# bab2min/Kiwi

Measured on AMD Instinct MI355X. Metric: sentences/sec on batched analyze(), device kernels with inputs resident in HBM (dictionary scan + lattice + Viterbi/Knlm, top-1); host-to-host rate: see e2e, higher is better.
Workload: dtype int32+f32; 1 GPU; c2-64k: 65536 synthetic sentences ({'exact_jamo': 40}), synthetic 'full' model (kiwi_amd/synth.py), Knlm, top-1; sentences_per_gpu=65536, chunks_per_gpu=65536, jamo_per_gpu=2621440, parallelism=shard1, device_bytes=9402884427, rerun_chunks=0

## Files before the change

### kiwi_amd/csrc/engine.hip

```cpp
#include <hip/hip_runtime.h>
#include <unistd.h>
#include <cstdio>
#include <cstring>
#include <ctime>
#include <algorithm>
#include <atomic>
#include <cstdlib>
#include <chrono>
#include <condition_variable>
#include <functional>
#include <map>
#include <mutex>
#include <numeric>
#include <stdexcept>
#include <thread>
#include "engine.hpp"
#include "pretok.hpp"
#include "hostpool.hpp"
#include "post_fast.hpp"
#include "viterbi_kernel.hpp"
#include "exact_math.hpp"
#include "cong_global.hpp"
#include "chr_freq.hpp"
#include "typo_lattice_kernel.hpp"
// ... 31 lines not shown
				size_t best = blocks.size();
				for (size_t i = 0; i < blocks.size(); ++i)
					if (blocks[i].device == device && blocks[i].cap >= n && blocks[i].cap <= 2 * n + (1u << 20) && (best == blocks.size() || blocks[i].cap < blocks[best].cap)) best = i;
				if (best == blocks.size()) return nullptr;
				void* p = blocks[best].p; capOut = blocks[best].cap; bytes -= capOut;
				blocks.erase(blocks.begin() + best);
				return p;
			}
			void give(void* p, size_t cap, int device)
			{
				{
					std::lock_guard<std::mutex> g{ mu };
					if (blocks.size() < kMaxBlocks && bytes + cap <= kMaxBytes) { blocks.push_back(Block{ p, cap, device }); bytes += cap; return; }
				}
				release(Block{ p, cap, device });
			}
			void trim()
			{
				std::lock_guard<std::mutex> g{ mu };
				for (auto& b : blocks) release(b);
				blocks.clear(); bytes = 0;
			}
		};
		DevBlockCache& devCache() { static DevBlockCache c; return c; }
		int currentDevice() { int d = 0; (void)hipGetDevice(&d); return d; }

		struct DevBuf
		{
			void* p = nullptr; size_t cap = 0; int device = 0;
			DevBuf() = default;
			DevBuf(const DevBuf&) = delete;
			DevBuf& operator=(const DevBuf&) = delete;
			~DevBuf() { release(); }
			void release() { if (p) devCache().give(p, cap, device); p = nullptr; cap = 0; }
			void ensure(size_t n)
			{
				if (n <= cap) return;
				release();
				device = currentDevice();
				const size_t want = n + n / 8 + 256;
				p = devCache().take(want, cap, device);
				if (!p)
				{
					hipError_t e = hipMalloc(&p, want);
					if (e == hipErrorOutOfMemory) { (void)hipGetLastError(); devCache().trim(); e = hipMalloc(&p, want); }
					if (e != hipSuccess) { p = nullptr; (void)hipGetLastError(); throw std::runtime_error{ std::string{ "HIP error in hipMalloc(" } + std::to_string(want) + " bytes): " + hipGetErrorString(e) }; }
					cap = want;
// ... 2363 lines not shown
```

### kiwi_amd/csrc/viterbi_pos.inc

```
#if !defined(KAMD_SBG) && !defined(KAMD_CONGG)
	template<int G> struct PosCaps
	{
#ifdef KAMD_TEST_SMALL_CAPS
		static constexpr uint32_t PST_CAP = 8;
#else
		static constexpr uint32_t PST_CAP = G == 16 ? 64 : 32;
#endif
		static constexpr uint32_t PHR = G == 16 ? 32 : 16;
	};
	constexpr uint32_t PBIG_CAP = 64;
	struct PosGroupCtx { uint64_t st, recs, uniq, nodeTypo; uint32_t stCap, stTop, posStart, ringTop, firstRec, retry, ofNodes, pad; };
	static_assert(sizeof(PosGroupCtx) == 64, "PosGroupCtx");
	template<int G> struct PosLayT
	{
		static constexpr uint32_t PST_CAP = PosCaps<G>::PST_CAP, PHR = PosCaps<G>::PHR;
		static constexpr uint32_t RBEG = 0, REND = 4 * RING, RCUM = 8 * RING;
		static constexpr uint32_t NCNT = 12 * RING;
		static constexpr uint32_t ACUR = NCNT + 4 * G, ALAST = ACUR + 32, ATMP = ALAST + 32;
#ifdef KAMD_TEST_DEAD_WINDOW
		static constexpr uint32_t DWIN_BITS = KAMD_TEST_DEAD_WINDOW;
#else
		static constexpr uint32_t DWIN_BITS = 256;
#endif
		static constexpr uint32_t DWIN = ATMP + 32, DWIN_WORDS = DWIN_BITS / 32;
		static constexpr uint32_t GCTX = DWIN + (G == 16 ? 32 : 0);
		static constexpr uint32_t RINFO = GCTX + 64;
		static constexpr uint32_t PBEST = RINFO;
		static constexpr uint32_t OVFL = RINFO + 4 * G;
		static constexpr uint32_t RECS = OVFL + 16;
		static constexpr uint32_t STSC = RECS + G * 48;
		static constexpr uint32_t STB = STSC + 4 * PST_CAP;
		static constexpr uint32_t HOTR = (STB + 2 * PST_CAP + 15) & ~15u;
		static constexpr uint32_t TYPR = HOTR + 16 * PHR;
#ifdef KAMD_CONG
// ... 80 lines not shown
	}
	__device__ __forceinline__ uint32_t nthSetBit(uint32_t v, uint32_t k)
	{
		uint32_t pos = 0, c;
		c = (uint32_t)__popc(v & 0xFFFFu); if (k >= c) { k -= c; pos += 16; v >>= 16; }
		c = (uint32_t)__popc(v & 0xFFu); if (k >= c) { k -= c; pos += 8; v >>= 8; }
		c = (uint32_t)__popc(v & 0xFu); if (k >= c) { k -= c; pos += 4; v >>= 4; }
		c = (uint32_t)__popc(v & 0x3u); if (k >= c) { k -= c; pos += 2; v >>= 2; }
		if (k >= (v & 1u)) pos += 1;
		return pos;
	}
	__device__ __forceinline__ void ldsMaxF(LDS_AS float* p, float v)
	{
#if defined(__HIP_DEVICE_COMPILE__)
		__hip_atomic_fetch_max(p, v, __ATOMIC_RELAXED, __HIP_MEMORY_SCOPE_WAVEFRONT);
#else
		uint32_t o = __atomic_load_n((uint32_t*)p, __ATOMIC_RELAXED);
		while (v > __uint_as_float(o) && !__atomic_compare_exchange_n((uint32_t*)p, &o, __float_as_uint(v), false, __ATOMIC_RELAXED, __ATOMIC_RELAXED)) {}
#endif
	}

	struct PosKernArgs { ModelView M; BatchView B; WorkView W; SearchParams P; const uint32_t* chunkOrder; uint32_t nWork; TYPO_ONLY(const float* nodeTypoAll;) CONG_ONLY(CongDev CG;) };
#ifdef KAMD_HIPEMU
	__device__ __noinline__ bool continueChunk(const PosKernArgs* A, uint32_t chunk, uint32_t gl, uint32_t grp, uint32_t slot, uint32_t resumeAt, const uint8_t* scratchCheck, const uint32_t* orderCheck, uint32_t nWorkCheck)
	{
#else
	__device__ __noinline__ bool continueChunk(uint32_t chunk, uint32_t gl, uint32_t grp, uint32_t slot, uint32_t resumeAt, const uint8_t* scratchCheck, const uint32_t* orderCheck, uint32_t nWorkCheck)
	{
		const PosKernArgs* A = (const PosKernArgs*)((const uint8_t*)__builtin_amdgcn_implicitarg_ptr() - ((sizeof(PosKernArgs) + 7) & ~(size_t)7));
#endif
		if (A->W.posScratch != scratchCheck || A->chunkOrder != orderCheck || A->nWork != nWorkCheck) return false;
		const ModelView& M = A->M; const SearchParams& P = A->P; const BatchView& B = A->B; const WorkView& W = A->W;
		CONG_ONLY(const CongDev& CG = A->CG;)
		GroupCtx<16> X(M, P);
		X.gl = gl; X.gshift = grp * 16; X.lds = grp * Lay<16>::SIZE;
		X.scratch = reinterpret_cast<GroupScratch*>(W.posScratch) + slot;
		X.tl = nullptr;
		TYPO_ONLY(X.typoAll = A->nodeTypoAll; X.nodeTypo = nullptr;)
		CONG_ONLY(X.CG = &CG; X.outFirst = false;)
		searchChunk<16>(X, B, W, chunk, resumeAt);
		return true;
	}

	template<int G, int WPS>
	__global__ void __launch_bounds__(64, WPS) k_pos_path(ModelView M, BatchView B, WorkView W, SearchParams P, const uint32_t* chunkOrder, uint32_t nWork TYPO_ONLY(, const float* nodeTypoAll) CONG_ONLY(, CongDev CGv))
	{
		static_assert(G == 16 || G == 8, "a lane group is one DPP row or half of one");
		using PosLay = PosLayT<G>;
		constexpr uint32_t NG = 64 / G, GM = (1u << G) - 1u, PST_CAP = PosLay::PST_CAP, PHR = PosLay::PHR;
		constexpr bool kLiveOnly = G == 16;
#ifdef KAMD_TYPO
		constexpr uint32_t kP = 2;
#else
		constexpr uint32_t kP = 16 / G;
#endif
		const uint32_t lane = threadIdx.x, gl = lane & (uint32_t)(G - 1), gshift = lane & (uint32_t)(64 - G), grp = lane / (uint32_t)G, lds = grp * PosLay::SIZE;
		const uint32_t il = lane & 15u, irow = lane >> 4;
		LDS_AS uint32_t* rBeg = ldsPtr<uint32_t>(lds + PosLay::RBEG);
		LDS_AS uint32_t* rEnd = ldsPtr<uint32_t>(lds + PosLay::REND);
		LDS_AS uint32_t* rCum = ldsPtr<uint32_t>(lds + PosLay::RCUM);
		LDS_AS uint32_t* nCnt = ldsPtr<uint32_t>(lds + PosLay::NCNT);
		LDS_AS uint32_t* aCur = ldsPtr<uint32_t>(lds + PosLay::ACUR);
		LDS_AS uint32_t* aLast = ldsPtr<uint32_t>(lds + PosLay::ALAST);
		LDS_AS uint32_t* aTmp = ldsPtr<uint32_t>(lds + PosLay::ATMP);
// ... 16 lines not shown
#define GBALLOT(p) ((uint32_t)((__ballot(p) >> gshift) & GM))
#define GSHFL(v, l) __shfl((v), (int)(l), G)
#ifdef KAMD_HIPEMU
#define WBALLOT(p) hipemu_ballot64(p)
#define WSHFL(v, l) hipemu_shfl64((v), (int)(l))
#define WREADLANE(v, l) hipemu_shfl64((v), (int)(l))
#define IROR(N, v) ((uint32_t)hipemu_row_ror64((int)(v), (N)))
#define IRORF(N, v) __uint_as_float((uint32_t)hipemu_row_ror64((int)__float_as_uint(v), (N)))
#else
#define WBALLOT(p) ((unsigned long long)__ballot(p))
#define WSHFL(v, l) __shfl((v), (int)(l), 64)
#define WREADLANE(v, l) ((uint32_t)__builtin_amdgcn_readlane((int)(v), (int)(l)))
#define IROR(N, v) rowRor<N>(v)
#define IRORF(N, v) rowRorF<N>(v)
#endif
#ifdef KAMD_POS_DEBUG
#define PBEACON(code, a, b2, c2) { if (W.beacon && mine && gl == 0) { uint32_t* bq_ = W.beacon + 64ull * chunk; __builtin_nontemporal_store((uint32_t)(code), bq_); __builtin_nontemporal_store((uint32_t)(a), bq_ + 1); __builtin_nontemporal_store((uint32_t)(b2), bq_ + 2); __builtin_nontemporal_store((uint32_t)(c2), bq_ + 3); } }
		unsigned long long tlLast = clock64(); uint32_t tlAcc[14] = { 0, 0, 0, 0, 0, 0, 0, 0, 0, 0, 0, 0, 0, 0 };
#define PTL(k) { const unsigned long long t_ = clock64(); tlAcc[k] += (uint32_t)(t_ - tlLast); tlLast = t_; }
#else
#define PBEACON(code, a, b2, c2)
#define PTL(k)
#endif
		const unsigned long long lowerMask64 = (1ull << lane) - 1ull;

		const uint32_t ci = blockIdx.x * NG + grp;
		const bool mine = ci < nWork;
		const uint32_t chunk = mine ? chunkOrder[ci] : chunkOrder[0];
		DevChunkResult* res = &W.results[chunk];
		bool active = mine && res->status == CS_OK;
		if (mine && !active && gl == 0) res->nPaths = 0;
		const bool searching = active;
		PBEACON(1, ci, 0, 0)
		const uint32_t nBase = W.nodeBase[chunk];
		const uint32_t Gn = W.nNodes[chunk];
		DevState* st = W.states + W.stateBase[chunk];
		const uint32_t stCap = (uint32_t)(W.stateBase[chunk + 1] - W.stateBase[chunk]);
		uint32_t* nodeStOff = W.nodeStateOff + nBase; uint32_t* nodeStCnt = W.nodeStateCnt + nBase; uint16_t* nodeLive = W.tmpIdx + 2ull * nBase;
		const uint8_t* uniq = B.spStates + B.spOff[chunk];
		uint8_t* reach = W.reach + nBase;
		const PosDesc* desc = W.posDesc + nBase;
		const PosRec* recs = W.posRecs + W.packBase[chunk];
		const uint32_t* posPrev = W.posPrev + nBase;
#ifdef KAMD_TYPO
		const float* nodeTypo = nodeTypoAll + nBase;
#else
		const float* nodeTypo = nullptr;
#endif
		const uint32_t nPos = active ? desc[0].firstRec : 0u, eosStart = active ? desc[0].pad2 : 0u;
		const uint32_t* posStarts = W.posMask + nBase;
		TYPO_ONLY(const uint32_t* posStarts2 = posStarts + W.nodeBase[B.nChunks];)
		const bool canPropagate = nPos <= 255 && active && desc[0].nNodes == 0;
		bool scanned = false;
		if (gl < 8) { aCur[gl] = gl == 0 ? 1u : 0u; aLast[gl] = 0; if constexpr (kLiveOnly) ldsPtr<uint32_t>(lds + PosLay::DWIN)[gl] = 0; }
		for (uint32_t k = gl; k < 16; k += G) gctx[k] = 0;
		rinfo[gl] = 0; if (gl == 0) *ovfL = 0;

		uint32_t stTop = 1, cumLive = 1;
		uint32_t ringTop = 1;
		uint32_t stopAt = 0;
		if (active)
		{
			if (gl == 0)
			{
				const MorphRec m0 = M.morphs[0];
				storeState(st, 0, M.h.bosNode, 0.f, 0.f, 0, m0.feat, COMMON_ROOT, 0, 0, m0.prevFlags, 0, 0xFFFFFFFFu, 0, 0.f, 0, 0);
				nodeStOff[0] = 0; nodeStCnt[0] = 1; nodeLive[0] = 1;
				rBeg[0] = 0; rEnd[0] = 1; rCum[0] = 1;
				ldsStore4(hotR, make_uint4((uint32_t)M.h.bosNode, 0u, (uint32_t)m0.feat | ((uint32_t)COMMON_ROOT << 16), (uint32_t)m0.prevFlags << 8));
				typR[0] = 0.f;
#ifdef KAMD_CONG
				ctxR[0] = 0;
#else
				const uint32_t c1 = M.lmChain[2 * (uint32_t)M.h.bosNode], c2 = M.lmChain[2 * (uint32_t)M.h.bosNode + 1];
				chR[0] = c1; chR[1] = c2;
				*reinterpret_cast<uint2*>(&st[0].pad0) = make_uint2(c1, c2);
#endif
			}
			for (uint32_t k = gl; k < Gn; k += G) reach[k] = k == 0 ? 1 : 0;
			if (!nPos) { stopAt = 1u | (8u << 24); active = false; }
		}

		uint4 dqA = make_uint4(0, 0, 0, 0), dqB = make_uint4(0, 0, 0, 0);
		uint32_t ppA = 0, rqA = 0;
		uint4 recA0 = make_uint4(0, 0, 0, 0), recA1 = recA0, recA2 = recA0, recB0 = recA0, recB1 = recA0, recB2 = recA0;
		if (active)
		{
			dqA = *reinterpret_cast<const uint4*>(desc + 1);
			if (nPos >= 2) dqB = *reinterpret_cast<const uint4*>(desc + 2);
			if (gl < ((dqA.x >> 16) & 0xFFu)) ppA = posPrev[(dqA.x & 0xFFFFu) + gl];
			if (gl < (dqA.z & 0xFFFFu)) rqA = recs[dqA.y + gl].rq;
			if constexpr (WPS <= 2) if (gl < (dqA.z & 0xFFFFu)) { const uint4* rp0 = reinterpret_cast<const uint4*>(recs + dqA.y + gl); recA0 = rp0[0]; recA1 = rp0[1]; recA2 = rp0[2]; }
		}

		uint32_t pi = 1, attempt = 0, retry0 = 0, retry1 = 0;
		uint4 dqC = make_uint4(0, 0, 0, 0); uint32_t ppB = 0, rqB = 0;
		uint32_t guardSteps = 0;
		__syncthreads();

		while (WBALLOT(active))
		{
			if (++guardSteps > 4u * 0x10000u) break;
			if (lane == 0) PSTAT(0, 1)
			if (gl == 0 && active) PSTAT(1, 1)
			const uint4 dq = dqA;
			const uint32_t i0 = dq.x & 0xFFFFu, m = (dq.x >> 16) & 0xFFu, firstRec = dq.y, nRec = dq.z & 0xFFFFu;
			uint32_t Qp[kP]; uint32_t rqp[kP], pBegRp[kP];
#pragma unroll
			for (uint32_t ps_ = 0; ps_ < kP; ++ps_) { Qp[ps_] = 0; rqp[ps_] = 0; pBegRp[ps_] = 0; }
			uint32_t posStart = stTop;
			CONG_ONLY(uint32_t ofNodes = 0;)
			uint4 rec0 = recA0, rec1 = recA1, rec2 = recA2;
			if (active)
			{
				PBEACON(2, pi, i0, (m << 16) | nRec)
				PTL(0)
				if ((dq.x >> 24) || m > (uint32_t)G || nRec > kP * (uint32_t)G) { stopAt = i0 | (1u << 24); active = false; }
			}
			if (active)
			{
				if (!attempt)
				{
					dqC = make_uint4(0, 0, 0, 0); ppB = 0; rqB = 0;
					if (pi + 2 <= nPos) dqC = *reinterpret_cast<const uint4*>(desc + pi + 2);
					if (pi + 1 <= nPos)
					{
						if (gl < ((dqB.x >> 16) & 0xFFu)) ppB = posPrev[(dqB.x & 0xFFFFu) + gl];
						if (gl < (dqB.z & 0xFFFFu)) rqB = recs[dqB.y + gl].rq;
						if constexpr (WPS <= 2) if (gl < (dqB.z & 0xFFFFu)) { const uint4* rp0 = reinterpret_cast<const uint4*>(recs + dqB.y + gl); recB0 = rp0[0]; recB1 = rp0[1]; recB2 = rp0[2]; }
					}
				}
				if constexpr (WPS > 2) if (gl < nRec) { const uint4* rp0 = reinterpret_cast<const uint4*>(recs + firstRec + gl); rec0 = rp0[0]; rec1 = rp0[1]; rec2 = rp0[2]; }
				rqp[0] = rqA;
				if constexpr (kP > 1) if (nRec > (uint32_t)G && gl + G < nRec) rqp[kP - 1] = recs[firstRec + G + gl].rq;
				uint32_t pBeg = 0, nP = 0, nLv = 0; bool bad = false; uint32_t why = 0;
				if (gl < m)
				{
					const uint32_t fp = ppA & 0xFFFFu, lp = fp + ((ppA >> 16) & 0xFFu);
					if (i0 + gl - fp + 1 >= RING) { bad = true; why = 2; }
					else
					{
						pBeg = rBeg[fp & (RING - 1)];
						nP = rEnd[lp & (RING - 1)] - pBeg;
						const uint32_t nLive = rCum[lp & (RING - 1)] - (fp ? rCum[(fp - 1) & (RING - 1)] : 0u);
						if (nLive > P.smallMax) { bad = true; why = 3; }
						nLv = nLive;
					}
				}
				nCnt[gl] = 0;
				if (gl == 0) { PHIST(0, nRec) PHIST(1, m) }
#pragma unroll
				for (uint32_t ps_ = 0; ps_ < kP; ++ps_)
				{
					const uint32_t rq = rqp[ps_];
					const uint32_t nlR = (rq >> 8) & 0xFFu, Rr = rq & 0xFFu;
					const uint32_t nPk = GSHFL(kLiveOnly ? nLv : nP, nlR), pBegR = GSHFL(pBeg, nlR);
					const uint32_t Q = ps_ * G + gl < nRec ? nPk * Rr : 0u;
#if defined(KAMD_POSSTATS) && defined(KAMD_HIPEMU)
					{ const uint32_t nAll = GSHFL(nP, nlR); if (kLiveOnly && ps_ * G + gl < nRec && !bad) PSTAT(5, (nAll - nPk) * Rr) }
#endif
					if (Q > PBIG_CAP || pBegR >= (1u << 27)) { bad = true; why = 4; }
					Qp[ps_] = Q; pBegRp[ps_] = pBegR;
					if (ps_ * G + gl < nRec) PHIST(3, Q)
				}
				if (gl < m && !bad) PHIST(5, i0 + gl - (ppA & 0xFFFFu))
				if (GBALLOT(bad)) { stopAt = i0 | (grpMaxU<G>(why) << 24); active = false; }
#ifdef KAMD_CONG
				if (active)
				{
					uint32_t wantL = 0;
#pragma unroll
					for (uint32_t ps_ = 0; ps_ < kP; ++ps_)
					{
						const uint32_t rq = rqp[ps_], nlR = (rq >> 8) & 0xFFu;
						const uint32_t nPk = GSHFL(nP, nlR);
						if (ps_ * G + gl < nRec && (rq & PR_OUT_FIRST) && nPk >= 4) wantL |= 1u << nlR;
					}
					const uint32_t want = grpOr<G>(wantL);
					for (uint32_t wn = want; wn; wn &= wn - 1)
					{
						const uint32_t j = (uint32_t)__ffs((int)wn) - 1u;
						const uint32_t pb = GSHFL(pBeg, j), np = GSHFL(nP, j);
						if (G < 16 || np > 16)
						{
							static_assert(4 * PBIG_CAP <= G * 48, "context list in the record area");
							LDS_AS uint32_t* cxs = ldsPtr<uint32_t>(lds + PosLay::RECS);
							for (uint32_t b = 0; b < np; b += G)
							{
								const uint32_t k = b + gl;
								if (k < np) { const Hot h = loadHot(st, pb + k); cxs[k] = (!h.dead() && !h.socket()) ? st[pb + k].pad0 : 0xFFFFFFFFu; }
							}
							waveSyncLds();
							uint32_t mu = 0;
							for (uint32_t b = 0; b < np; b += G)
							{
								const uint32_t k = b + gl;
								bool isNew = false;
								if (k < np)
								{
									const uint32_t cx = cxs[k];
									isNew = cx != 0xFFFFFFFFu;
// ... 7 lines not shown
						}
						if constexpr (G == 16)
						{
						uint32_t cx = 0xFFFFFFFFu; bool ok = false;
						if (gl < np) { const Hot h = loadHot(st, pb + gl); ok = !h.dead() && !h.socket(); cx = st[pb + gl].pad0; }
						const uint32_t okw = ok ? 1u : 0u;
						bool isNew = ok;
#define KAMD_UNIQ_STEP(N) { const uint32_t oc = rowRor<N>(cx), oo = rowRor<N>(okw); isNew = isNew & !((oo != 0) & (oc == cx) & (((gl - N) & 15u) < gl)); }
						KAMD_UNIQ_STEP(1) KAMD_UNIQ_STEP(2) KAMD_UNIQ_STEP(3) KAMD_UNIQ_STEP(4) KAMD_UNIQ_STEP(5) KAMD_UNIQ_STEP(6) KAMD_UNIQ_STEP(7) KAMD_UNIQ_STEP(8)
						KAMD_UNIQ_STEP(9) KAMD_UNIQ_STEP(10) KAMD_UNIQ_STEP(11) KAMD_UNIQ_STEP(12) KAMD_UNIQ_STEP(13) KAMD_UNIQ_STEP(14) KAMD_UNIQ_STEP(15)
#undef KAMD_UNIQ_STEP
						const uint32_t mu = (uint32_t)__popc(GBALLOT(isNew));
						if (mu >= 4 && mu != 8) ofNodes |= 1u << j;
						}
					}
				}
#endif
				if (active)
				{
					rinfo[gl] = pBegRp[0] | ((rqp[0] & 0xFFu) << 27);
					if (gl < nRec) { ldsStore4(lds + PosLay::RECS + 48 * gl, rec0); ldsStore4(lds + PosLay::RECS + 48 * gl + 16, rec1); ldsStore4(lds + PosLay::RECS + 48 * gl + 32, rec2); }
					if (gl == 0)
					{
						LDS_AS uint64_t* g64 = (LDS_AS uint64_t*)gctx;
						g64[0] = (uint64_t)st; g64[1] = (uint64_t)(recs + firstRec); g64[2] = (uint64_t)uniq; g64[3] = (uint64_t)nodeTypo;
						gctx[8] = stCap; gctx[9] = stTop; gctx[10] = stTop; gctx[11] = ringTop; gctx[12] = 0; gctx[13] = retry0 | (retry1 << 16);
#ifdef KAMD_CONG
						gctx[14] = ofNodes;
#else
						gctx[14] = 0;
#endif
						gctx[15] = 0;
						*ovfL = 0;
					}
					posStart = stTop;
				}
				PTL(1)
			}
			__syncthreads();

			for (uint32_t pass = 0; pass < kP; ++pass)
			{
			if (pass)
			{
				if (!WBALLOT(active && nRec > (uint32_t)G)) break;
				if (active)
				{
					rinfo[gl] = pBegRp[kP - 1] | ((rqp[kP - 1] & 0xFFu) << 27);
					if (G + gl < nRec)
					{
						const uint4* rp0 = reinterpret_cast<const uint4*>(recs + firstRec + G + gl);
						ldsStore4(lds + PosLay::RECS + 48 * gl, rp0[0]); ldsStore4(lds + PosLay::RECS + 48 * gl + 16, rp0[1]); ldsStore4(lds + PosLay::RECS + 48 * gl + 32, rp0[2]);
					}
				}
				__syncthreads();
			}
			const uint32_t Qw = active ? ((kP > 1 && pass) ? Qp[kP - 1] : Qp[0]) : 0u;

			{
				uint32_t S16 = Qw;
				{ uint32_t t; t = IROR(1, S16); S16 += il >= 1 ? t : 0u; t = IROR(2, S16); S16 += il >= 2 ? t : 0u; t = IROR(4, S16); S16 += il >= 4 ? t : 0u; t = IROR(8, S16); S16 += il >= 8 ? t : 0u; }
				const uint32_t T0 = WREADLANE(S16, 15), T1 = WREADLANE(S16, 31), T2 = WREADLANE(S16, 47);
				const uint32_t Winc = S16 + (irow >= 1 ? T0 : 0u) + (irow >= 2 ? T1 : 0u) + (irow >= 3 ? T2 : 0u);
				const unsigned long long nzAll = WBALLOT(Qw != 0);
				uint32_t recDoneW = 0, baseW = 0, guardW = 0;
				while (recDoneW < 64)
				{
					const unsigned long long nz = nzAll & ~((1ull << recDoneW) - 1ull);
					if (!nz) break;
					if (++guardW > 80u) { *ovfL = 1; break; }
					const bool take = lane >= recDoneW && Winc - baseW <= 64u;
					const uint32_t n = (uint32_t)__popcll(WBALLOT(take));
					if (!n) { *ovfL = 1; break; }
					const uint32_t nItems = WREADLANE(Winc, recDoneW + n - 1) - baseW;
// ... 382 lines not shown
				}
				waveSyncLds();
				const bool scanRoots = GBALLOT(otherRoot) != 0;
				for (uint32_t b = 0; b < cnt; b += G)
				{
					const uint32_t i = b + gl;
					if (i >= cnt) continue;
					const uint32_t bits = stB[i]; const float lim = stSc[i] + P.cutOff;
					bool kill = lim < pbest[(bits >> 8) & 0xFu];
					if (scanRoots && (bits & 0x1Fu))
					{
						kill = false;
						for (uint32_t j = 0; j < cnt; ++j)
						{
							const uint32_t bj = stB[j];
							if (!(bj & SB_MORPH_SOCKET) && (bj & 0xF1Fu) == (bits & 0xF1Fu) && lim < stSc[j]) kill = true;
						}
					}
					if constexpr (kLiveOnly)
					{
						LDS_AS uint32_t* dwp = ldsPtr<uint32_t>(lds + PosLay::DWIN) + (((posStart + i) >> 5) & (PosLay::DWIN_WORDS - 1u));
						if (kill) ldsOr(dwp, 1u << ((posStart + i) & 31u)); else ldsAnd(dwp, ~(1u << ((posStart + i) & 31u)));
					}
					if (kill) { st[posStart + i].dead = 1; if (ringTop - (posStart + i) <= PHR) ldsPtr<uint32_t>(hotR + 16 * ((posStart + i) & (PHR - 1)) + 12)[0] |= 1u << 16; }
					ldsAdd(&nCnt[(bits >> 8) & 0xFu], 1u | ((bits & PSB_PASS1) ? 0u : 1u << 8) | (kill ? 0u : 1u << 16) | ((kill || (bits & SB_STATE_SOCKET)) ? 0u : 1u << 24));
				}
				waveSyncLds();
				PTL(8)
				const uint32_t myC = nCnt[gl];
				const uint32_t myCnt = myC & 0xFFu, myP0 = (myC >> 8) & 0xFFu, myLive = (myC >> 16) & 0xFFu, myFree = myC >> 24;
				const bool isNode = gl < m, formNode = isNode && !((dq.z >> (16 + gl)) & 1u);
				bool redo = false;
				if (attempt == 0)
				{
					const uint32_t lacking = GBALLOT(isNode && !myP0);
					if (lacking) { retry0 = lacking; attempt = 1; redo = true; }
				}
				if (!redo && attempt <= 1)
				{
					const uint32_t stateless = GBALLOT(isNode && !myCnt && ((dq.w >> gl) & 1u));
					if (stateless) { retry0 |= stateless; retry1 = stateless; attempt = 2; redo = true; }
				}
				if (redo && gl == 0) PSTAT(13, 1)
				if (redo) stTop = posStart;
				else
				{
				const uint32_t spJ = ppA >> 24;
// ... 3 lines not shown
				if (!nonFree) flagBits = GBALLOT(isNode && (formNode || tbit(aLast, spJ)));
				else
				{
					if (!canPropagate) { stopAt = i0 | (9u << 24); active = false; }
					else
					{
					const bool predFlag = isNode && tbit(aCur, spJ);
					flagBits = 0; bool disconnected = false;
					for (uint32_t j = 0; j < m; ++j)
					{
						const uint32_t spj = GSHFL(spJ, j);
						if (!((nonFree >> j) & 1u))
						{
							if (!((dq.z >> (16 + j)) & 1u) || tbit(aLast, spj)) flagBits |= 1u << j;
							continue;
						}
						const uint32_t later = GBALLOT(predFlag && gl > j);
						if (gl < 8) aTmp[gl] = aCur[gl];
						waveSyncLds();
						if (flagBits || later) sbit(aTmp, pi);
						for (uint32_t x = pi + 1; x <= nPos; x += G)
						{
							uint32_t st4 = 0; TYPO_ONLY(uint32_t st8 = 0;)
							if (x + gl <= nPos) { st4 = posStarts[x + gl]; TYPO_ONLY(st8 = posStarts2[x + gl];) }
							const uint32_t nx = nPos - x + 1 < (uint32_t)G ? nPos - x + 1 : (uint32_t)G;
							for (uint32_t t = 0; t < nx; ++t)
							{
								const uint32_t s4 = GSHFL(st4, t);
								uint32_t reached = tbit(aTmp, s4 & 0xFFu) | tbit(aTmp, (s4 >> 8) & 0xFFu) | tbit(aTmp, (s4 >> 16) & 0xFFu) | tbit(aTmp, s4 >> 24);
								TYPO_ONLY({ const uint32_t s8 = GSHFL(st8, t); reached |= tbit(aTmp, s8 & 0xFFu) | tbit(aTmp, (s8 >> 8) & 0xFFu) | tbit(aTmp, (s8 >> 16) & 0xFFu) | tbit(aTmp, s8 >> 24); })
								if (reached) sbit(aTmp, x + t);
							}
						}
						if (!tbit(aTmp, eosStart)) { disconnected = true; break; }
						waveSyncLds();
						if (gl < 8) aLast[gl] = aTmp[gl];
						waveSyncLds();
						scanned = true;
					}
					if (disconnected) { stopAt = i0 | (7u << 24); active = false; }
					}
				}

				if (active)
				{
				if (flagBits) sbit(aCur, pi);
				PTL(9)
				PBEACON(10, pi, cnt, 0)
				const uint32_t inclBoth = grpScan<G>(isNode ? (myCnt | (myLive << 16)) : 0u, gl);
				const uint32_t inclCnt = inclBoth & 0xFFFFu, inclLive = inclBoth >> 16;
				if (isNode)
				{
					const uint32_t i = i0 + gl, ns = posStart + inclCnt - myCnt;
					rBeg[i & (RING - 1)] = ns; rEnd[i & (RING - 1)] = ns + myCnt; rCum[i & (RING - 1)] = cumLive + inclLive;
					nodeStOff[i] = ns; nodeStCnt[i] = myCnt; nodeLive[i] = (uint16_t)myLive;
#ifdef KAMD_POS_TRACE
					fprintf(stderr, "commit pi %u node %u ns %u cnt %u live %u free %u p0 %u attempt %u\n", pi, i, ns, myCnt, myLive, myFree, myP0, attempt);
#endif
					reach[i] = (uint8_t)((flagBits >> gl) & 1u);
				}
				cumLive += GSHFL(inclLive, G - 1);
				dqA = dqB; dqB = dqC; ppA = ppB; rqA = rqB; recA0 = recB0; recA1 = recB1; recA2 = recB2;
				++pi; attempt = 0; retry0 = 0; retry1 = 0;
				waveSyncLds();
				PTL(10)
				if (pi > nPos)
				{
			{
				const uint4 enq = reinterpret_cast<const uint4*>(W.nodes + nBase + (Gn - 1))[0];
				const uint32_t enPrev = enq.z & 0xFFFFu, enNPrev = W.nodes[nBase + Gn - 1].nPrev;
				const uint32_t firstPrev = Gn - 1 - enPrev;
				const uint32_t pBegE = nodeStOff[firstPrev];
				const uint32_t nPE = (enPrev && enNPrev) ? nodeStOff[firstPrev + enNPrev - 1] + nodeStCnt[firstPrev + enNPrev - 1] - pBegE : 0u;
				EndCand* endBuf = reinterpret_cast<EndCand*>(st + stTop);
				const uint64_t freeBytes = (uint64_t)(stCap - stTop) * sizeof(DevState);
				const uint32_t endCap = freeBytes > (uint64_t)Gn * 4 ? (uint32_t)((freeBytes - (uint64_t)Gn * 4) / sizeof(EndCand)) : 0u;
				const bool openEnding = (B.chunkFlags[chunk] & 1) != 0;
				const uint32_t nUniq = B.spOff[chunk + 1] - B.spOff[chunk];
				uint32_t nEnd = 0; bool endOverflow = false;
				for (uint32_t pb = 0; pb < nPE; pb += G)
				{
					const uint32_t p = pb + gl;
					bool ok = false; float c = 0, first = 0, ptypo = 0; uint8_t pRoot = 0, pSp = 0;
					if (p < nPE)
					{
						const uint4* ps4 = reinterpret_cast<const uint4*>(st + pBegE + p);
						const uint4 a = ps4[0], b2 = ps4[1];
						const MorphRec pm = M.morphs[b2.w];
						const uint8_t pSocket = (uint8_t)a.w, pDead = (uint8_t)(a.w >> 16);
						pRoot = (uint8_t)(a.z >> 16); pSp = (uint8_t)(a.z >> 24); ptypo = __uint_as_float(b2.x);
						ok = !pSocket && !pDead;
						if (ok && !(pm.flags & MF_SINGLE) && pm.nChunks <= (pm.socket ? 2u : 1u) && pm.vowel != CV_NONE) ok = false;
						if (ok && pm.tag == T_Z_SIOT) ok = false;
						if (ok)
						{
							c = __uint_as_float(a.y);
							if (!openEnding)
							{
								int32_t ln = (int32_t)a.x;
#ifdef KAMD_CONG
								uint32_t ectx = ps4[2].z;
// ... 5 lines not shown
								if (pSp & 1) c -= 2;
								if (pSp & 2) c -= 2;
							}
						}
					}
					const uint32_t mult = (ok && pRoot == COMMON_ROOT) ? nUniq : (ok ? 1u : 0u);
					const uint32_t incl = grpScan<G>(mult, gl);
					const uint32_t baseE = nEnd + incl - mult;
					for (uint32_t r = 0; r < mult; ++r)
					{
						if (baseE + r < endCap)
						{
							EndCand e; e.score = c; e.fcs = first; e.typo = ptypo; e.parent = pBegE + p; e.pad = 0;
							if (pRoot == COMMON_ROOT) { e.rootId = (uint8_t)r; e.sp = uniq[r]; } else { e.rootId = pRoot; e.sp = pSp; }
							endBuf[baseE + r] = e;
						}
						else endOverflow = true;
					}
					nEnd += GSHFL(incl, G - 1);
				}
				const bool anyOverflow = GBALLOT(endOverflow) != 0;
				if (gl == 0)
				{
					res->nEnd = nEnd; res->endOff = stTop; res->nPaths = 0;
					res->status = anyOverflow ? CS_ERR_STATE_OVERFLOW : CS_OK;
					res->pad = kPosChunkDone;
				}
			}
					active = false;
				}
				}
				}
			}
			__syncthreads();
		}

		if (searching && stopAt && scanned)
			for (uint32_t k = (stopAt & 0xFFFFFFu) + gl; k + 1 < Gn; k += G) reach[k] = (uint8_t)tbit(aLast, posPrev[k] >> 24);
		PBEACON(11, stopAt, 0, 0)
#ifdef KAMD_POS_DEBUG
		PTL(11)
		if (W.beacon && mine && gl == 0) { volatile uint32_t* bq_ = W.beacon + 64ull * chunk; for (int k_ = 0; k_ < 14; ++k_) bq_[16 + k_] = tlAcc[k_]; bq_[31] = nPos; }
#endif
		const bool handOver = searching && stopAt != 0;
		bool cont = false;
		uint32_t slot = 0xFFFFFFFFu;
		if (W.posScratch)
		{
			if (handOver) { if (gl == 0) slot = atomicAdd(W.posContCounter, 1u); slot = GSHFL(slot, 0); }
			cont = handOver && slot < W.posContSlots;
		}
		if constexpr (G == 8)
		{
			const unsigned long long cm = WBALLOT(cont && gl == 0);
			if (cm)
			{
				__syncthreads();
				LDS_AS uint32_t* lst = ldsPtr<uint32_t>(PosLay::ROWMAP);
				static_assert(Lay<16>::TOTAL <= PosLayT<8>::ROWMAP && 3 * 4 * (64 / 8) <= 128, "list of the chunks carried on");
				if (cont && gl == 0) { const uint32_t at = (uint32_t)__popcll(cm & lowerMask64); lst[3 * at] = chunk; lst[3 * at + 1] = stopAt; lst[3 * at + 2] = slot; }
				const uint32_t nH = (uint32_t)__popcll(cm);
				LDS_AS float* lb = ldsPtr<float>(Lay<16>::LB);
				for (uint32_t t = lane; t < 2 * T_MAX + 1; t += 64)
				{
					float v = 0;
					if (t == 2 * T_MAX) v = 5.f;
					else if (t < T_MAX) { if (t == T_NNP || t == T_NP || t == T_IC) v = -1; else if (t == T_SB) v = -3; }
					else { const uint8_t r = (uint8_t)(t - T_MAX); v = (isEClass(r) || isJClass(r) || isSuffixTag(r) || r == T_VCP) ? -1.f : 0.f; }
					lb[t] = v;
				}
				__syncthreads();
#ifdef KAMD_HIPEMU
				hipemu_set_width(16);
#endif
				for (uint32_t base = 0; base < nH; base += 4)
				{
					const uint32_t e = base + irow;
					if (e < nH)
					{
						const uint32_t chunkE = lst[3 * e], stopE = lst[3 * e + 1], slotE = lst[3 * e + 2];
#ifdef KAMD_HIPEMU
						const PosKernArgs A{ M, B, W, P, chunkOrder, nWork TYPO_ONLY(, nodeTypoAll) CONG_ONLY(, CGv) };
						const bool ok = continueChunk(&A, chunkE, il, irow, slotE, stopE & 0xFFFFFFu, W.posScratch, chunkOrder, nWork);
#else
						const bool ok = continueChunk(chunkE, il, irow, slotE, stopE & 0xFFFFFFu, W.posScratch, chunkOrder, nWork);
#endif
						if (il == 0)
						{
							if (ok) W.results[chunkE].pad = kPosChunkDone | (stopE & 0xFF000000u);
							else { W.results[chunkE].pad = stopE; *W.posHandOver = 1; }
						}
					}
				}
#ifdef KAMD_HIPEMU
				hipemu_set_width(8);
#endif
			}
			if (handOver && !cont && gl == 0) { res->pad = stopAt; *W.posHandOver = 1; }
		}
		else
		{
		if (WBALLOT(cont))
		{
			__syncthreads();
			LDS_AS float* lb = ldsPtr<float>(Lay<16>::LB);
			for (uint32_t t = lane; t < 2 * T_MAX + 1; t += 64)
			{
				float v = 0;
				if (t == 2 * T_MAX) v = 5.f;
				else if (t < T_MAX) { if (t == T_NNP || t == T_NP || t == T_IC) v = -1; else if (t == T_SB) v = -3; }
				else { const uint8_t r = (uint8_t)(t - T_MAX); v = (isEClass(r) || isJClass(r) || isSuffixTag(r) || r == T_VCP) ? -1.f : 0.f; }
				lb[t] = v;
			}
			__syncthreads();
			if (cont)
			{
#ifdef KAMD_HIPEMU
				const PosKernArgs A{ M, B, W, P, chunkOrder, nWork TYPO_ONLY(, nodeTypoAll) CONG_ONLY(, CGv) };
				cont = continueChunk(&A, chunk, gl, grp, slot, stopAt & 0xFFFFFFu, W.posScratch, chunkOrder, nWork);
#else
				cont = continueChunk(chunk, gl, grp, slot, stopAt & 0xFFFFFFu, W.posScratch, chunkOrder, nWork);
#endif
				if (cont && gl == 0) res->pad = kPosChunkDone | (stopAt & 0xFF000000u);
			}
		}
		if (handOver && !cont && gl == 0) { res->pad = stopAt; *W.posHandOver = 1; }
		}
#undef GBALLOT
#undef GSHFL
#undef WBALLOT
#undef WSHFL
#undef WREADLANE
#undef IROR
#undef IRORF
#undef PBEACON
#undef PTL
#undef PSTAT
#undef PHIST
	}
#endif
```

Baseline: 14.11 million sentences/s.

## Cut live registers in POS Viterbi kernel by spilling chunk pointers to LDS

```diff
diff --git a/kiwi_amd/csrc/engine.hip b/kiwi_amd/csrc/engine.hip
--- a/kiwi_amd/csrc/engine.hip
+++ b/kiwi_amd/csrc/engine.hip
@@ -77,7 +77,7 @@
 				blocks.clear(); bytes = 0;
 			}
 		};
-		DevBlockCache& devCache() { static DevBlockCache c; return c; }
+		DevBlockCache& devCache() { static DevBlockCache* c = new DevBlockCache; return *c; }
 		int currentDevice() { int d = 0; (void)hipGetDevice(&d); return d; }
 
 		struct DevBuf
diff --git a/kiwi_amd/csrc/viterbi_pos.inc b/kiwi_amd/csrc/viterbi_pos.inc
--- a/kiwi_amd/csrc/viterbi_pos.inc
+++ b/kiwi_amd/csrc/viterbi_pos.inc
@@ -9,7 +9,7 @@
 		static constexpr uint32_t PHR = G == 16 ? 32 : 16;
 	};
 	constexpr uint32_t PBIG_CAP = 64;
-	struct PosGroupCtx { uint64_t st, recs, uniq, nodeTypo; uint32_t stCap, stTop, posStart, ringTop, firstRec, retry, ofNodes, pad; };
+	struct PosGroupCtx { uint64_t st, recs, uniq, nodeTypo; uint32_t stCap, stTop, posStart, ringTop, chunk, retry, ofNodes, nNodes; };
 	static_assert(sizeof(PosGroupCtx) == 64, "PosGroupCtx");
 	template<int G> struct PosLayT
 	{
@@ -136,14 +136,18 @@
 
 	struct PosKernArgs { ModelView M; BatchView B; WorkView W; SearchParams P; const uint32_t* chunkOrder; uint32_t nWork; TYPO_ONLY(const float* nodeTypoAll;) CONG_ONLY(CongDev CG;) };
 #ifdef KAMD_HIPEMU
-	__device__ __noinline__ bool continueChunk(const PosKernArgs* A, uint32_t chunk, uint32_t gl, uint32_t grp, uint32_t slot, uint32_t resumeAt, const uint8_t* scratchCheck, const uint32_t* orderCheck, uint32_t nWorkCheck)
-	{
-#else
-	__device__ __noinline__ bool continueChunk(uint32_t chunk, uint32_t gl, uint32_t grp, uint32_t slot, uint32_t resumeAt, const uint8_t* scratchCheck, const uint32_t* orderCheck, uint32_t nWorkCheck)
+	__device__ __noinline__ void continueChunk(const PosKernArgs* A, uint32_t chunk, uint32_t gl, uint32_t grp, uint32_t slot, uint32_t stopAt, const uint8_t* scratchCheck, const uint32_t* orderCheck, uint32_t nWorkCheck)
+	{
+#else
+	__device__ __noinline__ void continueChunk(uint32_t chunk, uint32_t gl, uint32_t grp, uint32_t slot, uint32_t stopAt, const uint8_t* scratchCheck, const uint32_t* orderCheck, uint32_t nWorkCheck)
 	{
 		const PosKernArgs* A = (const PosKernArgs*)((const uint8_t*)__builtin_amdgcn_implicitarg_ptr() - ((sizeof(PosKernArgs) + 7) & ~(size_t)7));
 #endif
-		if (A->W.posScratch != scratchCheck || A->chunkOrder != orderCheck || A->nWork != nWorkCheck) return false;
+		if (A->W.posScratch != scratchCheck || A->chunkOrder != orderCheck || A->nWork != nWorkCheck)
+		{
+			if (gl == 0) { A->W.results[chunk].pad = stopAt; *A->W.posHandOver = 1; }
+			return;
+		}
 		const ModelView& M = A->M; const SearchParams& P = A->P; const BatchView& B = A->B; const WorkView& W = A->W;
 		CONG_ONLY(const CongDev& CG = A->CG;)
 		GroupCtx<16> X(M, P);
@@ -152,8 +156,8 @@
 		X.tl = nullptr;
 		TYPO_ONLY(X.typoAll = A->nodeTypoAll; X.nodeTypo = nullptr;)
 		CONG_ONLY(X.CG = &CG; X.outFirst = false;)
-		searchChunk<16>(X, B, W, chunk, resumeAt);
-		return true;
+		searchChunk<16>(X, B, W, chunk, stopAt & 0xFFFFFFu);
+		if (gl == 0) W.results[chunk].pad = kPosChunkDone | (stopAt & 0xFF000000u);
 	}
 
 	template<int G, int WPS>
@@ -216,38 +220,52 @@
 #define PBEACON(code, a, b2, c2)
 #define PTL(k)
 #endif
+		constexpr int kWaitVm0 = (0 << 0) | (0 << 14) | (7 << 4) | (15 << 8);
+#if defined(__HIP_DEVICE_COMPILE__)
+#define POS_LOADS_ARRIVED() __builtin_amdgcn_s_waitcnt(kWaitVm0)
+#else
+#define POS_LOADS_ARRIVED() (void)0
+#endif
 		const unsigned long long lowerMask64 = (1ull << lane) - 1ull;
 
 		const uint32_t ci = blockIdx.x * NG + grp;
 		const bool mine = ci < nWork;
 		const uint32_t chunk = mine ? chunkOrder[ci] : chunkOrder[0];
-		DevChunkResult* res = &W.results[chunk];
-		bool active = mine && res->status == CS_OK;
-		if (mine && !active && gl == 0) res->nPaths = 0;
+		bool active = mine && W.results[chunk].status == CS_OK;
+		if (mine && !active && gl == 0) W.results[chunk].nPaths = 0;
 		const bool searching = active;
 		PBEACON(1, ci, 0, 0)
 		const uint32_t nBase = W.nodeBase[chunk];
 		const uint32_t Gn = W.nNodes[chunk];
-		DevState* st = W.states + W.stateBase[chunk];
 		const uint32_t stCap = (uint32_t)(W.stateBase[chunk + 1] - W.stateBase[chunk]);
-		uint32_t* nodeStOff = W.nodeStateOff + nBase; uint32_t* nodeStCnt = W.nodeStateCnt + nBase; uint16_t* nodeLive = W.tmpIdx + 2ull * nBase;
-		const uint8_t* uniq = B.spStates + B.spOff[chunk];
-		uint8_t* reach = W.reach + nBase;
-		const PosDesc* desc = W.posDesc + nBase;
-		const PosRec* recs = W.posRecs + W.packBase[chunk];
-		const uint32_t* posPrev = W.posPrev + nBase;
-#ifdef KAMD_TYPO
-		const float* nodeTypo = nodeTypoAll + nBase;
-#else
-		const float* nodeTypo = nullptr;
-#endif
-		const uint32_t nPos = active ? desc[0].firstRec : 0u, eosStart = active ? desc[0].pad2 : 0u;
-		const uint32_t* posStarts = W.posMask + nBase;
-		TYPO_ONLY(const uint32_t* posStarts2 = posStarts + W.nodeBase[B.nChunks];)
-		const bool canPropagate = nPos <= 255 && active && desc[0].nNodes == 0;
+		const uint32_t recBase = W.packBase[chunk];
+		auto nodeStOff = [&](uint32_t i) -> uint32_t& { return W.nodeStateOff[nBase + i]; };
+		auto nodeStCnt = [&](uint32_t i) -> uint32_t& { return W.nodeStateCnt[nBase + i]; };
+		auto nodeLive = [&](uint32_t i) -> uint16_t& { return W.tmpIdx[2ull * nBase + i]; };
+		auto reach = [&](uint32_t i) -> uint8_t& { return W.reach[nBase + i]; };
+		auto desc = [&](uint32_t i) -> const PosDesc& { return W.posDesc[nBase + i]; };
+		auto posPrev = [&](uint32_t i) -> const uint32_t& { return W.posPrev[nBase + i]; };
+		auto posStarts = [&](uint32_t i) -> const uint32_t& { return W.posMask[nBase + i]; };
+		auto recs = [&](uint32_t i) -> const PosRec& { return W.posRecs[recBase + i]; };
+		auto stArena = [&]() -> DevState* { return reinterpret_cast<DevState*>(((LDS_AS uint64_t*)gctx)[0]); };
+		auto uniqStates = [&]() -> const uint8_t* { return reinterpret_cast<const uint8_t*>(((LDS_AS uint64_t*)gctx)[2]); };
+		const uint32_t nPos = active ? desc(0).firstRec : 0u, eosStart = active ? desc(0).pad2 : 0u;
+		TYPO_ONLY(const uint32_t nBase2 = nBase + W.nodeBase[B.nChunks];)
+		const bool canPropagate = nPos <= 255 && active && desc(0).nNodes == 0;
 		bool scanned = false;
 		if (gl < 8) { aCur[gl] = gl == 0 ? 1u : 0u; aLast[gl] = 0; if constexpr (kLiveOnly) ldsPtr<uint32_t>(lds + PosLay::DWIN)[gl] = 0; }
-		for (uint32_t k = gl; k < 16; k += G) gctx[k] = 0;
+		if (gl == 0)
+		{
+			LDS_AS uint64_t* g64 = (LDS_AS uint64_t*)gctx;
+			for (uint32_t k = 8; k < 16; ++k) gctx[k] = 0;
+			gctx[12] = chunk; gctx[15] = Gn;
+			g64[0] = (uint64_t)(W.states + W.stateBase[chunk]); g64[1] = 0; g64[2] = (uint64_t)(B.spStates + B.spOff[chunk]);
+#ifdef KAMD_TYPO
+			g64[3] = (uint64_t)(nodeTypoAll + nBase);
+#else
+			g64[3] = 0;
+#endif
+		}
 		rinfo[gl] = 0; if (gl == 0) *ovfL = 0;
 
 		uint32_t stTop = 1, cumLive = 1;
@@ -258,8 +276,9 @@
 			if (gl == 0)
 			{
 				const MorphRec m0 = M.morphs[0];
+				DevState* st = W.states + W.stateBase[chunk];
 				storeState(st, 0, M.h.bosNode, 0.f, 0.f, 0, m0.feat, COMMON_ROOT, 0, 0, m0.prevFlags, 0, 0xFFFFFFFFu, 0, 0.f, 0, 0);
-				nodeStOff[0] = 0; nodeStCnt[0] = 1; nodeLive[0] = 1;
+				nodeStOff(0) = 0; nodeStCnt(0) = 1; nodeLive(0) = 1;
 				rBeg[0] = 0; rEnd[0] = 1; rCum[0] = 1;
 				ldsStore4(hotR, make_uint4((uint32_t)M.h.bosNode, 0u, (uint32_t)m0.feat | ((uint32_t)COMMON_ROOT << 16), (uint32_t)m0.prevFlags << 8));
 				typR[0] = 0.f;
@@ -271,7 +290,7 @@
 				*reinterpret_cast<uint2*>(&st[0].pad0) = make_uint2(c1, c2);
 #endif
 			}
-			for (uint32_t k = gl; k < Gn; k += G) reach[k] = k == 0 ? 1 : 0;
+			for (uint32_t k = gl; k < Gn; k += G) reach(k) = k == 0 ? 1 : 0;
 			if (!nPos) { stopAt = 1u | (8u << 24); active = false; }
 		}
 
@@ -280,16 +299,17 @@
 		uint4 recA0 = make_uint4(0, 0, 0, 0), recA1 = recA0, recA2 = recA0, recB0 = recA0, recB1 = recA0, recB2 = recA0;
 		if (active)
 		{
-			dqA = *reinterpret_cast<const uint4*>(desc + 1);
-			if (nPos >= 2) dqB = *reinterpret_cast<const uint4*>(desc + 2);
-			if (gl < ((dqA.x >> 16) & 0xFFu)) ppA = posPrev[(dqA.x & 0xFFFFu) + gl];
-			if (gl < (dqA.z & 0xFFFFu)) rqA = recs[dqA.y + gl].rq;
-			if constexpr (WPS <= 2) if (gl < (dqA.z & 0xFFFFu)) { const uint4* rp0 = reinterpret_cast<const uint4*>(recs + dqA.y + gl); recA0 = rp0[0]; recA1 = rp0[1]; recA2 = rp0[2]; }
+			dqA = *reinterpret_cast<const uint4*>(&desc(1));
+			if (nPos >= 2) dqB = *reinterpret_cast<const uint4*>(&desc(2));
+			if (gl < ((dqA.x >> 16) & 0xFFu)) ppA = posPrev((dqA.x & 0xFFFFu) + gl);
+			if (gl < (dqA.z & 0xFFFFu)) rqA = recs(dqA.y + gl).rq;
+			if constexpr (WPS <= 2) if (gl < (dqA.z & 0xFFFFu)) { const uint4* rp0 = reinterpret_cast<const uint4*>(&recs(dqA.y + gl)); recA0 = rp0[0]; recA1 = rp0[1]; recA2 = rp0[2]; }
 		}
 
 		uint32_t pi = 1, attempt = 0, retry0 = 0, retry1 = 0;
 		uint4 dqC = make_uint4(0, 0, 0, 0); uint32_t ppB = 0, rqB = 0;
 		uint32_t guardSteps = 0;
+		POS_LOADS_ARRIVED();
 		__syncthreads();
 
 		while (WBALLOT(active))
@@ -313,20 +333,20 @@
 			}
 			if (active)
 			{
+				if constexpr (WPS > 2) if (gl < nRec) { const uint4* rp0 = reinterpret_cast<const uint4*>(&recs(firstRec + gl)); rec0 = rp0[0]; rec1 = rp0[1]; rec2 = rp0[2]; }
+				rqp[0] = rqA;
+				if constexpr (kP > 1) if (nRec > (uint32_t)G && gl + G < nRec) rqp[kP - 1] = recs(firstRec + G + gl).rq;
 				if (!attempt)
 				{
 					dqC = make_uint4(0, 0, 0, 0); ppB = 0; rqB = 0;
-					if (pi + 2 <= nPos) dqC = *reinterpret_cast<const uint4*>(desc + pi + 2);
+					if (pi + 2 <= nPos) dqC = *reinterpret_cast<const uint4*>(&desc(pi + 2));
 					if (pi + 1 <= nPos)
 					{
-						if (gl < ((dqB.x >> 16) & 0xFFu)) ppB = posPrev[(dqB.x & 0xFFFFu) + gl];
-						if (gl < (dqB.z & 0xFFFFu)) rqB = recs[dqB.y + gl].rq;
-						if constexpr (WPS <= 2) if (gl < (dqB.z & 0xFFFFu)) { const uint4* rp0 = reinterpret_cast<const uint4*>(recs + dqB.y + gl); recB0 = rp0[0]; recB1 = rp0[1]; recB2 = rp0[2]; }
-					}
-				}
-				if constexpr (WPS > 2) if (gl < nRec) { const uint4* rp0 = reinterpret_cast<const uint4*>(recs + firstRec + gl); rec0 = rp0[0]; rec1 = rp0[1]; rec2 = rp0[2]; }
-				rqp[0] = rqA;
-				if constexpr (kP > 1) if (nRec > (uint32_t)G && gl + G < nRec) rqp[kP - 1] = recs[firstRec + G + gl].rq;
+						if (gl < ((dqB.x >> 16) & 0xFFu)) ppB = posPrev((dqB.x & 0xFFFFu) + gl);
+						if (gl < (dqB.z & 0xFFFFu)) rqB = recs(dqB.y + gl).rq;
+						if constexpr (WPS <= 2) if (gl < (dqB.z & 0xFFFFu)) { const uint4* rp0 = reinterpret_cast<const uint4*>(&recs(dqB.y + gl)); recB0 = rp0[0]; recB1 = rp0[1]; recB2 = rp0[2]; }
+					}
+				}
 				uint32_t pBeg = 0, nP = 0, nLv = 0; bool bad = false; uint32_t why = 0;
 				if (gl < m)
 				{
@@ -371,6 +391,7 @@
 						if (ps_ * G + gl < nRec && (rq & PR_OUT_FIRST) && nPk >= 4) wantL |= 1u << nlR;
 					}
 					const uint32_t want = grpOr<G>(wantL);
+					const DevState* st = want ? stArena() : nullptr;
 					for (uint32_t wn = want; wn; wn &= wn - 1)
 					{
 						const uint32_t j = (uint32_t)__ffs((int)wn) - 1u;
@@ -424,21 +445,19 @@
 					if (gl < nRec) { ldsStore4(lds + PosLay::RECS + 48 * gl, rec0); ldsStore4(lds + PosLay::RECS + 48 * gl + 16, rec1); ldsStore4(lds + PosLay::RECS + 48 * gl + 32, rec2); }
 					if (gl == 0)
 					{
-						LDS_AS uint64_t* g64 = (LDS_AS uint64_t*)gctx;
-						g64[0] = (uint64_t)st; g64[1] = (uint64_t)(recs + firstRec); g64[2] = (uint64_t)uniq; g64[3] = (uint64_t)nodeTypo;
-						gctx[8] = stCap; gctx[9] = stTop; gctx[10] = stTop; gctx[11] = ringTop; gctx[12] = 0; gctx[13] = retry0 | (retry1 << 16);
+						gctx[8] = stCap; gctx[9] = stTop; gctx[10] = stTop; gctx[11] = ringTop; gctx[13] = retry0 | (retry1 << 16);
 #ifdef KAMD_CONG
 						gctx[14] = ofNodes;
 #else
 						gctx[14] = 0;
 #endif
-						gctx[15] = 0;
 						*ovfL = 0;
 					}
 					posStart = stTop;
 				}
 				PTL(1)
 			}
+			if constexpr (WPS > 2) POS_LOADS_ARRIVED();
 			__syncthreads();
 
 			for (uint32_t pass = 0; pass < kP; ++pass)
@@ -451,7 +470,7 @@
 					rinfo[gl] = pBegRp[kP - 1] | ((rqp[kP - 1] & 0xFFu) << 27);
 					if (G + gl < nRec)
 					{
-						const uint4* rp0 = reinterpret_cast<const uint4*>(recs + firstRec + G + gl);
+						const uint4* rp0 = reinterpret_cast<const uint4*>(&recs(firstRec + G + gl));
 						ldsStore4(lds + PosLay::RECS + 48 * gl, rp0[0]); ldsStore4(lds + PosLay::RECS + 48 * gl + 16, rp0[1]); ldsStore4(lds + PosLay::RECS + 48 * gl + 32, rp0[2]);
 					}
 				}
@@ -880,7 +899,7 @@
 						LDS_AS uint32_t* dwp = ldsPtr<uint32_t>(lds + PosLay::DWIN) + (((posStart + i) >> 5) & (PosLay::DWIN_WORDS - 1u));
 						if (kill) ldsOr(dwp, 1u << ((posStart + i) & 31u)); else ldsAnd(dwp, ~(1u << ((posStart + i) & 31u)));
 					}
-					if (kill) { st[posStart + i].dead = 1; if (ringTop - (posStart + i) <= PHR) ldsPtr<uint32_t>(hotR + 16 * ((posStart + i) & (PHR - 1)) + 12)[0] |= 1u << 16; }
+					if (kill) { stArena()[posStart + i].dead = 1; if (ringTop - (posStart + i) <= PHR) ldsPtr<uint32_t>(hotR + 16 * ((posStart + i) & (PHR - 1)) + 12)[0] |= 1u << 16; }
 					ldsAdd(&nCnt[(bits >> 8) & 0xFu], 1u | ((bits & PSB_PASS1) ? 0u : 1u << 8) | (kill ? 0u : 1u << 16) | ((kill || (bits & SB_STATE_SOCKET)) ? 0u : 1u << 24));
 				}
 				waveSyncLds();
@@ -930,7 +949,7 @@
 						for (uint32_t x = pi + 1; x <= nPos; x += G)
 						{
 							uint32_t st4 = 0; TYPO_ONLY(uint32_t st8 = 0;)
-							if (x + gl <= nPos) { st4 = posStarts[x + gl]; TYPO_ONLY(st8 = posStarts2[x + gl];) }
+							if (x + gl <= nPos) { st4 = posStarts(x + gl); TYPO_ONLY(st8 = W.posMask[nBase2 + x + gl];) }
 							const uint32_t nx = nPos - x + 1 < (uint32_t)G ? nPos - x + 1 : (uint32_t)G;
 							for (uint32_t t = 0; t < nx; ++t)
 							{
@@ -961,11 +980,11 @@
 				{
 					const uint32_t i = i0 + gl, ns = posStart + inclCnt - myCnt;
 					rBeg[i & (RING - 1)] = ns; rEnd[i & (RING - 1)] = ns + myCnt; rCum[i & (RING - 1)] = cumLive + inclLive;
-					nodeStOff[i] = ns; nodeStCnt[i] = myCnt; nodeLive[i] = (uint16_t)myLive;
+					nodeStOff(i) = ns; nodeStCnt(i) = myCnt; nodeLive(i) = (uint16_t)myLive;
 #ifdef KAMD_POS_TRACE
 					fprintf(stderr, "commit pi %u node %u ns %u cnt %u live %u free %u p0 %u attempt %u\n", pi, i, ns, myCnt, myLive, myFree, myP0, attempt);
 #endif
-					reach[i] = (uint8_t)((flagBits >> gl) & 1u);
+					reach(i) = (uint8_t)((flagBits >> gl) & 1u);
 				}
 				cumLive += GSHFL(inclLive, G - 1);
 				dqA = dqB; dqB = dqC; ppA = ppB; rqA = rqB; recA0 = recB0; recA1 = recB1; recA2 = recB2;
@@ -975,16 +994,18 @@
 				if (pi > nPos)
 				{
 			{
-				const uint4 enq = reinterpret_cast<const uint4*>(W.nodes + nBase + (Gn - 1))[0];
+				const uint32_t chunkE = gctx[12], Gn = gctx[15];
+				const uint4 enq = reinterpret_cast<const uint4*>(&W.nodes[nBase + Gn - 1])[0];
 				const uint32_t enPrev = enq.z & 0xFFFFu, enNPrev = W.nodes[nBase + Gn - 1].nPrev;
 				const uint32_t firstPrev = Gn - 1 - enPrev;
-				const uint32_t pBegE = nodeStOff[firstPrev];
-				const uint32_t nPE = (enPrev && enNPrev) ? nodeStOff[firstPrev + enNPrev - 1] + nodeStCnt[firstPrev + enNPrev - 1] - pBegE : 0u;
+				const uint32_t pBegE = nodeStOff(firstPrev);
+				const uint32_t nPE = (enPrev && enNPrev) ? nodeStOff(firstPrev + enNPrev - 1) + nodeStCnt(firstPrev + enNPrev - 1) - pBegE : 0u;
+				DevState* st = stArena(); const uint8_t* uniq = uniqStates();
 				EndCand* endBuf = reinterpret_cast<EndCand*>(st + stTop);
 				const uint64_t freeBytes = (uint64_t)(stCap - stTop) * sizeof(DevState);
 				const uint32_t endCap = freeBytes > (uint64_t)Gn * 4 ? (uint32_t)((freeBytes - (uint64_t)Gn * 4) / sizeof(EndCand)) : 0u;
-				const bool openEnding = (B.chunkFlags[chunk] & 1) != 0;
-				const uint32_t nUniq = B.spOff[chunk + 1] - B.spOff[chunk];
+				const bool openEnding = (B.chunkFlags[chunkE] & 1) != 0;
+				const uint32_t nUniq = B.spOff[chunkE + 1] - B.spOff[chunkE];
 				uint32_t nEnd = 0; bool endOverflow = false;
 				for (uint32_t pb = 0; pb < nPE; pb += G)
 				{
@@ -1036,6 +1057,7 @@
 				const bool anyOverflow = GBALLOT(endOverflow) != 0;
 				if (gl == 0)
 				{
+					DevChunkResult* res = &W.results[chunkE];
 					res->nEnd = nEnd; res->endOff = stTop; res->nPaths = 0;
 					res->status = anyOverflow ? CS_ERR_STATE_OVERFLOW : CS_OK;
 					res->pad = kPosChunkDone;
@@ -1049,8 +1071,9 @@
 			__syncthreads();
 		}
 
+		const uint32_t chunkL = gctx[12], GnL = gctx[15];
 		if (searching && stopAt && scanned)
-			for (uint32_t k = (stopAt & 0xFFFFFFu) + gl; k + 1 < Gn; k += G) reach[k] = (uint8_t)tbit(aLast, posPrev[k] >> 24);
+			for (uint32_t k = (stopAt & 0xFFFFFFu) + gl; k + 1 < GnL; k += G) reach(k) = (uint8_t)tbit(aLast, posPrev(k) >> 24);
 		PBEACON(11, stopAt, 0, 0)
 #ifdef KAMD_POS_DEBUG
 		PTL(11)
@@ -1072,7 +1095,7 @@
 				__syncthreads();
 				LDS_AS uint32_t* lst = ldsPtr<uint32_t>(PosLay::ROWMAP);
 				static_assert(Lay<16>::TOTAL <= PosLayT<8>::ROWMAP && 3 * 4 * (64 / 8) <= 128, "list of the chunks carried on");
-				if (cont && gl == 0) { const uint32_t at = (uint32_t)__popcll(cm & lowerMask64); lst[3 * at] = chunk; lst[3 * at + 1] = stopAt; lst[3 * at + 2] = slot; }
+				if (cont && gl == 0) { const uint32_t at = (uint32_t)__popcll(cm & lowerMask64); lst[3 * at] = chunkL; lst[3 * at + 1] = stopAt; lst[3 * at + 2] = slot; }
 				const uint32_t nH = (uint32_t)__popcll(cm);
 				LDS_AS float* lb = ldsPtr<float>(Lay<16>::LB);
 				for (uint32_t t = lane; t < 2 * T_MAX + 1; t += 64)
@@ -1095,25 +1118,21 @@
 						const uint32_t chunkE = lst[3 * e], stopE = lst[3 * e + 1], slotE = lst[3 * e + 2];
 #ifdef KAMD_HIPEMU
 						const PosKernArgs A{ M, B, W, P, chunkOrder, nWork TYPO_ONLY(, nodeTypoAll) CONG_ONLY(, CGv) };
-						const bool ok = continueChunk(&A, chunkE, il, irow, slotE, stopE & 0xFFFFFFu, W.posScratch, chunkOrder, nWork);
-#else
-						const bool ok = continueChunk(chunkE, il, irow, slotE, stopE & 0xFFFFFFu, W.posScratch, chunkOrder, nWork);
-#endif
-						if (il == 0)
-						{
-							if (ok) W.results[chunkE].pad = kPosChunkDone | (stopE & 0xFF000000u);
-							else { W.results[chunkE].pad = stopE; *W.posHandOver = 1; }
-						}
+						continueChunk(&A, chunkE, il, irow, slotE, stopE, W.posScratch, chunkOrder, nWork);
+#else
+						continueChunk(chunkE, il, irow, slotE, stopE, W.posScratch, chunkOrder, nWork);
+#endif
 					}
 				}
 #ifdef KAMD_HIPEMU
 				hipemu_set_width(8);
 #endif
 			}
-			if (handOver && !cont && gl == 0) { res->pad = stopAt; *W.posHandOver = 1; }
+			if (handOver && !cont && gl == 0) { W.results[chunkL].pad = stopAt; *W.posHandOver = 1; }
 		}
 		else
 		{
+		if (handOver && !cont && gl == 0) { W.results[chunkL].pad = stopAt; *W.posHandOver = 1; }
 		if (WBALLOT(cont))
 		{
 			__syncthreads();
@@ -1131,15 +1150,14 @@
 			{
 #ifdef KAMD_HIPEMU
 				const PosKernArgs A{ M, B, W, P, chunkOrder, nWork TYPO_ONLY(, nodeTypoAll) CONG_ONLY(, CGv) };
-				cont = continueChunk(&A, chunk, gl, grp, slot, stopAt & 0xFFFFFFu, W.posScratch, chunkOrder, nWork);
-#else
-				cont = continueChunk(chunk, gl, grp, slot, stopAt & 0xFFFFFFu, W.posScratch, chunkOrder, nWork);
-#endif
-				if (cont && gl == 0) res->pad = kPosChunkDone | (stopAt & 0xFF000000u);
+				continueChunk(&A, chunkL, gl, grp, slot, stopAt, W.posScratch, chunkOrder, nWork);
+#else
+				continueChunk(chunkL, gl, grp, slot, stopAt, W.posScratch, chunkOrder, nWork);
+#endif
 			}
 		}
-		if (handOver && !cont && gl == 0) { res->pad = stopAt; *W.posHandOver = 1; }
 		}
+#undef POS_LOADS_ARRIVED
 #undef GBALLOT
 #undef GSHFL
 #undef WBALLOT
```

After: 14.92 million sentences/s, median of 6. +5.7%, better.
